# Kim-Dongjun/Soft-Truncation

Measured on AMD Instinct MI355X. Metric: training images/sec (DDPM++ CIFAR-10 32x32), higher is better.
Workload: dtype f32; 1 GPU; DDPM++ (VP) CIFAR-10 32x32, configs/vp/CIFAR10/ddpmpp_nll_st.py (BASELINE configs[1]); per_gpu_batch=128, global_batch=128, parallelism=dp1

## Files before the change

### soft-truncation_amd/csrc/conv.hip

```cpp
#include "igemm.h"
#include "stk_fp16.h"
#include "stk_fp16_train.h"

namespace {

using igemm::Cfg;
using igemm::MnMajor;
using igemm::keep_if;
using igemm::strip_row;

typedef __attribute__((address_space(1))) float gfloat;

struct ConvP {
  const float* x1; const float* x2; int C1, C2;
  const float* w; int w_layout;
  const float* bias; const float* temb; int temb_stride; const float* res; float inv_div; int use_div;
  float* y;
  const float* dy; float* dx1; float* dx2; float beta1, beta2, alpha;
  float* part; long part_stride;
  int N, H, W, Cin, Cout, OH, OW, KH, KW, stride, pad, sshift;
  int HW, OHW, taps;
  int ohw_shift, ow_shift;
};

// ... 561 lines not shown
  const bool al = stk_aligned16(p.part) && p.part_stride % 4 == 0 &&
                  (dgrad ? (p.HW % 4 == 0 && (!p.dx1 || stk_aligned16(p.dx1)) && (!p.dx2 || stk_aligned16(p.dx2)))
                         : (p.OHW % 4 == 0 && stk_aligned16(p.y) && (!p.res || stk_aligned16(p.res))));
  if (al && Ng % 4 == 0) {
    const dim3 rgrid((unsigned)stk_ew_grid((long)M * Ng / 4));
    if (dgrad) hipLaunchKernelGGL(slab_dgrad_kernel<4>, rgrid, dim3(256), 0, s, p, splits, M, (int)Ng);
    else hipLaunchKernelGGL(slab_fwd_kernel<4>, rgrid, dim3(256), 0, s, p, splits, M, (int)Ng);
  } else {
    const dim3 rgrid((unsigned)stk_ew_grid((long)M * Ng));
    if (dgrad) hipLaunchKernelGGL(slab_dgrad_kernel<1>, rgrid, dim3(256), 0, s, p, splits, M, (int)Ng);
    else hipLaunchKernelGGL(slab_fwd_kernel<1>, rgrid, dim3(256), 0, s, p, splits, M, (int)Ng);
  }
}

#include "conv_thin.h"
#include "conv_x2.h"
#include "conv_pl.h"
#include "conv_x2d.h"
#include "conv_x2w.h"

__device__ __forceinline__ long splitk_dst(long j, int layout, long CC, int Cout, int Cin, int taps) {
  if (layout == 0) {
    const int tap = (int)(j / CC);
    return (j - (long)tap * CC) * taps + tap;
  }
  const int co = (int)(j / Cin), ci = (int)(j - (long)co * Cin);
  return (long)ci * Cout + co;
}
__global__ __launch_bounds__(256) void splitk_reduce_kernel(const float* __restrict__ part, float* __restrict__ dw,
                                                            long n, int splits, long stride, float alpha, int layout,
                                                            int Cout, int Cin, int taps) {
  const long gstride = (long)gridDim.x * 256;
  const long CC = (long)Cout * Cin;
  const long n4 = ((n | stride) & 3) == 0 ? n / 4 : 0;
  for (long v = (long)blockIdx.x * 256 + threadIdx.x; v < n4; v += gstride) {
    const float4* src = reinterpret_cast<const float4*>(part) + v;
    float4 acc = {0.f, 0.f, 0.f, 0.f};
#pragma unroll 8
    for (int z = 0; z < splits; ++z) {
      const float4 t = src[(long)z * (stride / 4)];
      acc.x += t.x; acc.y += t.y; acc.z += t.z; acc.w += t.w;
    }
    const float a4[4] = {acc.x, acc.y, acc.z, acc.w};
#pragma unroll
    for (int e = 0; e < 4; ++e) dw[splitk_dst(4 * v + e, layout, CC, Cout, Cin, taps)] += alpha * a4[e];
  }
  for (long j = 4 * n4 + (long)blockIdx.x * 256 + threadIdx.x; j < n; j += gstride) {
    float sum = 0.f;
    for (int z = 0; z < splits; ++z) sum += part[(long)z * stride + j];
    dw[splitk_dst(j, layout, CC, Cout, Cin, taps)] += alpha * sum;
  }
}

__global__ __launch_bounds__(256) void splitk_reduce9_kernel(const float* __restrict__ part, float* __restrict__ dw, long CC,
                                                             int splits, long stride, float alpha) {
  __shared__ float s[256 * 9];
  const long q0 = (long)blockIdx.x * 256;
  const long q = q0 + threadIdx.x;
  const bool live = q < CC;
  float acc[9];
#pragma unroll
  for (int t = 0; t < 9; ++t) acc[t] = 0.f;
  const float* src = part + (live ? q : 0);
  int z = 0;
  for (; z + 4 <= splits; z += 4) {
    float v[4][9];
#pragma unroll
    for (int u = 0; u < 4; ++u)
#pragma unroll
      for (int t = 0; t < 9; ++t) v[u][t] = src[(long)(z + u) * stride + (long)t * CC];
#pragma unroll
    for (int u = 0; u < 4; ++u)
#pragma unroll
      for (int t = 0; t < 9; ++t) acc[t] += v[u][t];
  }
  for (; z < splits; ++z)
#pragma unroll
    for (int t = 0; t < 9; ++t) acc[t] += src[(long)z * stride + (long)t * CC];
#pragma unroll
  for (int t = 0; t < 9; ++t) s[threadIdx.x * 9 + t] = alpha * acc[t];
  __syncthreads();
  const long base = q0 * 9, end = CC * 9;
#pragma unroll
  for (int k = 0; k < 9; ++k) {
    const long i = base + k * 256 + threadIdx.x;
    if (i < end) dw[i] += s[k * 256 + threadIdx.x];
  }
}

template <int COLS>
__global__ __launch_bounds__(256) void wgrad9_kernel(ConvP p, int tiles_m, int tiles_n, int k_per_split) {
  constexpr int ROWS = 32 / COLS, TW = COLS + 2, TH = ROWS + 2, TSZ = TH * TW;
  constexpr int XS = TSZ | 1;
  constexpr int LDA = 129;
  constexpr int NX = (32 * TSZ + 255) / 256;
  constexpr int NA = 16;
  __shared__ float lds[32 * LDA + 32 * XS];
  float* As = lds;
  float* Xs = lds + 32 * LDA;

  const int tid = threadIdx.x, lane = tid & 63, wid = tid >> 6;
  const int fk = lane >> 5, fc = lane & 31;
  const int id = xcd_remap(blockIdx.x, gridDim.x);
  const int tn = id % tiles_n;
  const int rest = id / tiles_n;
  const int tm = rest % tiles_m, zs = rest / tiles_m;
// ... 252 lines not shown
    using A2 = std::conditional_t<X1, x2::ActLoader16<true, TAPS>, x2::ActLoader<true, TAPS>>;
    if (g.dual) hipLaunchKernelGGL((x2::gemm_kernel<A2, E>), g.grid, dim3(256), 0, g.s, g.p, g.q, g.M, g.Ng, g.tm, g.tn, g.nch,
                                   g.chunks_per_split, g.xpart, g.nx);
    else hipLaunchKernelGGL((x2::gemm_kernel<A1, E>), g.grid, dim3(256), 0, g.s, g.p, g.q, g.M, g.Ng, g.tm, g.tn, g.nch,
                            g.chunks_per_split, g.xpart, g.nx);
  } else if (g.halo) {
    if (g.p.W == 64)
      hipLaunchKernelGGL((x2d::gemm_halo_kernel<64, E, 1>), g.grid, dim3(256), 0, g.s, g.p, g.q, g.M, g.Ng, g.tm, g.tn, g.nch / 9, g.xpart, g.nx);
    else if (g.p.W == 32)
      hipLaunchKernelGGL((x2d::gemm_halo_kernel<32, E, 1>), g.grid, dim3(256), 0, g.s, g.p, g.q, g.M, g.Ng, g.tm, g.tn, g.nch / 9, g.xpart, g.nx);
    else
      hipLaunchKernelGGL((x2d::gemm_halo_kernel<16, E, 1>), g.grid, dim3(256), 0, g.s, g.p, g.q, g.M, g.Ng, g.tm, g.tn, g.nch / 9, g.xpart, g.nx);
  } else {
    hipLaunchKernelGGL((x2d::gemm_kernel<TAPS, 128, E>), g.grid, dim3(256), 0, g.s, g.p, g.q, g.M, g.Ng, g.tm, g.tn, g.nch,
                       g.chunks_per_split, g.xpart, g.nx);
  }
}
template <class E>
void split_gemm(const SplitGemm& g) {
  if (g.p.taps == 9) split_gemm_taps<E, 9>(g);
  else split_gemm_taps<E, 1>(g);
}

template <class EP>
int launch_split(ConvP p, const SplitPlan& r0, const float* s1, int S1, const float* s2, int S2, int M, long Ng, int dgrad,
                 void* ws, hipStream_t s, const void* wp_ready, float* amax, const void* planes, const float* planes_amax,
                 bool amax_valid, bool x1) {
  x2::Src q;
  q.s1 = s1; q.s2 = S2 > 0 ? s2 : s1; q.S1 = S1; q.S2 = S2; q.Kc = S1 + S2; q.Mpad = x2::pad128(M); q.taps = p.taps;
  q.pl = static_cast<const unsigned char*>(planes); q.pl_stride = planes ? pl::plane_bytes(p.N, S1, p.HW) : 0;
  const SplitWs lay = split_ws(r0, M, q.Kc, p.taps);
  unsigned char* base = reinterpret_cast<unsigned char*>(((uintptr_t)ws + 255) & ~(uintptr_t)255);
  float* xpart = reinterpret_cast<float*>(base + lay.xpart);
  p.part = reinterpret_cast<float*>(base + lay.part);
  p.part_stride = r0.slab;
  if (amax) xpart = amax + (dgrad ? 2 * x2::NPART : 0);
  if (planes) {
    xpart = const_cast<float*>(planes_amax);
  } else if (!(amax_valid && amax)) {
    hipLaunchKernelGGL(x2::amax_partial_kernel, dim3(x2::NPART), dim3(x2::AMAX_THREADS), 0, s, s1, (long)p.N * S1 * p.HW, xpart);
    if (S2 > 0)
      hipLaunchKernelGGL(x2::amax_partial_kernel, dim3(x2::NPART), dim3(x2::AMAX_THREADS), 0, s, s2, (long)p.N * S2 * p.HW,
                         xpart + x2::NPART);
    STK_CHECK_LAUNCH();
  }
  if (wp_ready) {
    q.wp = static_cast<const unsigned short*>(wp_ready);
  } else {
    x2::WprepDesc one = {};
    one.w = p.w; one.wp = base; one.M = M; one.Kc = q.Kc; one.Mpad = q.Mpad;
    one.taps = p.taps; one.flip = dgrad;
    split_weight_strides(p, dgrad, one.sm, one.sk);
    hipLaunchKernelGGL(x2::wamax_kernel, dim3(x2::WPART, 1), dim3(256), 0, s, nullptr, one);
    hipLaunchKernelGGL(x2::wprep_kernel, dim3((unsigned)stk_cdiv((long)q.Mpad * q.Kc, 256L)), dim3(256), 0, s, nullptr, one);
    STK_CHECK_LAUNCH();
    q.wp = reinterpret_cast<const unsigned short*>(base);
  }
  const int nch = planes && x1 ? p.taps * ((q.Kc / x2::KC + 1) / 2) : p.taps * (q.Kc / x2::KC);
  const SplitPlan r = planes && x1 ? x1_plan(r0, nch) : r0;
  SplitGemm g = {p, q, M, (int)Ng, q.Mpad / 128, stk_cdiv((int)Ng, 128), nch, r.chunks_per_split, xpart,
                 S2 > 0 ? 2 * x2::NPART : x2::NPART, S2 > 0, planes != nullptr, planes && x2d::halo_ok(p, p.taps, r0.splits),
                 dim3(), s};
  g.grid = dim3((unsigned)(g.tm * g.tn * r.splits));
  if (r0.splits == 1) {
    if (x1) split_gemm<OneProduct<EP>>(g);
    else split_gemm<EP>(g);
    STK_CHECK_LAUNCH();
    return STK_OK;
  }
  if (x1) split_gemm<OneProduct<EpSlab>>(g);
  else split_gemm<EpSlab>(g);
  STK_CHECK_LAUNCH();
  launch_slab_sum(p, r.splits, M, Ng, dgrad, s);
  STK_CHECK_LAUNCH();
  return STK_OK;
}

struct SplitWgradPlan { int ok; int splits; int chunks_per_split; long slab; int rows3; };
inline SplitWgradPlan split_wgrad_plan(int C1, int C2, int N, int Cout, int H, int W, int OH, int OW, int KH, int KW,
                                       int stride, int pad) {
  SplitWgradPlan q = {0, 0, 0, 0, 0};
  const int Cin = C1 + C2;
  const long K = (long)N * H * W;
  const int cmax = Cout > C1 ? (Cout > C2 ? Cout : C2) : (C1 > C2 ? C1 : C2);
  if (K * cmax * 4 >= 0x7fffffffL || (C2 > 0 && C1 % 32)) return q;
  const bool pow2 = (W & (W - 1)) == 0 && ((H * W) & (H * W - 1)) == 0;
  const bool geom = (KH == 3 && KW == 3 && pad == 1) || (KH == 1 && KW == 1 && pad == 0);
  if (!geom || stride != 1 || OH != H || OW != W || !pow2 || W < 4 || H * W < 16 || Cin < 64 || Cout < 64 ||
      K > 0x7fffffffL || K % 32)
    return q;
  const int taps = KH * KW;
  q.rows3 = (taps == 9 && W >= 8 && (C2 == 0 || C1 % 16 == 0)) ? 1 : 0;
  const long tiles = q.rows3 ? 3L * stk_cdiv(Cout, 128) * stk_cdiv(Cin, 64)
                             : (long)taps * stk_cdiv(Cout, 128) * stk_cdiv(Cin, 128);
  if (taps == 1 && tiles < 2) return q;
  const long chunks = K / 32;
  constexpr long w1_wgs = 256;
  long splits = (taps == 1 && tiles < 6 ? w1_wgs : 512) / tiles;
  if (splits > chunks / 8) splits = chunks / 8;
  if (splits < 1) splits = 1;
  q.chunks_per_split = (int)((chunks + splits - 1) / splits);
  q.splits = (int)((chunks + q.chunks_per_split - 1) / q.chunks_per_split);
  q.slab = (long)Cout * Cin * taps;
  q.ok = 1;
  return q;
}
template <int FORM>
// ... 480 lines not shown
                               false, f16x1);
}

int stk_conv2d_dgrad_pl_f32(const void* dypl, const float* dyamax, const float* w, int w_layout, float* dx1, int C1,
                            float beta1, float* dx2, int C2, float beta2, float alpha, int N, int H, int W, int Cout,
                            int KH, int KW, const void* wp, void* ws, long ws_bytes, void* stream) {
  return dgrad_pl_impl(dypl, dyamax, w, w_layout, dx1, C1, beta1, dx2, C2, beta2, alpha, N, H, W, Cout, KH, KW, wp, ws, ws_bytes,
                       stream, false);
}

int stk_conv2d_dgrad_pl_f16x1(const void* dypl, const float* dyamax, const float* w, int w_layout, float* dx1, int C1,
                              float beta1, float* dx2, int C2, float beta2, float alpha, int N, int H, int W, int Cout,
                              int KH, int KW, const void* wp, void* ws, long ws_bytes, void* stream) {
  return dgrad_pl_impl(dypl, dyamax, w, w_layout, dx1, C1, beta1, dx2, C2, beta2, alpha, N, H, W, Cout, KH, KW, wp, ws, ws_bytes,
                       stream, true);
}

int stk_conv2d_wgrad_pl_ok(int N, int H, int W, int Cin, int Cout) { return x2w::plan(N, H, W, Cin, Cout).ok; }

long stk_conv2d_wgrad_pl_ws_bytes(int N, int H, int W, int Cin, int Cout) {
  long m = 0;
  for (int wgs : {0, 256, 512, 768, 1024}) {
    const x2w::Plan q = x2w::plan(N, H, W, Cin, Cout, wgs);
    if (q.ok && (long)q.splits * q.slab > m) m = (long)q.splits * q.slab;
  }
  return m ? m * 4 + 256 : 0;
}

static int wgrad_pl_impl(const void* xpl, const float* xrec, const void* dypl, const float* dyrec, float* dw, float alpha,
                         float* ws, long ws_bytes, int N, int H, int W, int Cin, int Cout, int wgs, void* stream, bool f16x1) {
  if (!xpl || !xrec || !dypl || !dyrec || !dw || !ws || wgs < 0 || wgs > 1024) return STK_EINVAL;
  const x2w::Plan q = x2w::plan(N, H, W, Cin, Cout, wgs);
  if (!q.ok) return STK_EUNSUPPORTED;
  if (ws_bytes < (long)q.splits * q.slab * 4) return STK_EINVAL;
  x2w::Args a = {};
  a.dypl = static_cast<const unsigned char*>(dypl); a.dyrec = dyrec; a.dy_ps = pl::plane_bytes(N, Cout, H * W);
  a.xpl = static_cast<const unsigned char*>(xpl); a.xrec = xrec; a.x_ps = pl::plane_bytes(N, Cin, H * W);
  if (2 * a.dy_ps >= 0x7fffffffL || 2 * a.x_ps >= 0x7fffffffL) return STK_EUNSUPPORTED;
  a.part = ws; a.part_stride = q.slab;
  a.N = N; a.H = H; a.W = W; a.HW = H * W; a.Cin = Cin; a.Cout = Cout; a.Cob = Cout / 32; a.Cib = Cin / 32;
  a.tiles_co = stk_cdiv(Cout, 128); a.tiles_ci = Cin / 32;
  a.nchunks_total = (int)((long)N * H * W / 32); a.chunks_per_split = q.chunks_per_split;
  hipStream_t s = (hipStream_t)stream;
  const dim3 grid((unsigned)(a.tiles_co * a.tiles_ci * q.splits));
  if (f16x1) {
    if (q.groups == 2) launch_x2w<2 | x2w::X1_FORM>(a, W, grid, s);
    else launch_x2w<1 | x2w::X1_FORM>(a, W, grid, s);
  } else if (q.groups == 2) {
    launch_x2w<2>(a, W, grid, s);
  } else {
    launch_x2w<1>(a, W, grid, s);
  }
  STK_CHECK_LAUNCH();
  if (q.splits <= 64)
    hipLaunchKernelGGL(splitk_reduce9_kernel, dim3((unsigned)stk_cdiv((long)Cout * Cin, 256L)), dim3(256), 0, s, ws, dw, (long)Cout * Cin,
                       q.splits, q.slab, alpha);
  else
    hipLaunchKernelGGL(splitk_reduce_kernel, dim3(stk_ew_grid((q.slab + 3) / 4)), dim3(256), 0, s, ws, dw, q.slab, q.splits,
                       q.slab, alpha, 0, Cout, Cin, 9);
  STK_CHECK_LAUNCH();
  return STK_OK;
}

int stk_conv2d_wgrad_pl_f32(const void* xpl, const float* xrec, const void* dypl, const float* dyrec, float* dw,
                            float alpha, float* ws, long ws_bytes, int N, int H, int W, int Cin, int Cout, void* stream) {
  return stk_conv2d_wgrad_pl_wgs_f32(xpl, xrec, dypl, dyrec, dw, alpha, ws, ws_bytes, N, H, W, Cin, Cout, 0, stream);
}

int stk_conv2d_wgrad_pl_wgs_f32(const void* xpl, const float* xrec, const void* dypl, const float* dyrec, float* dw,
                                float alpha, float* ws, long ws_bytes, int N, int H, int W, int Cin, int Cout, int wgs, void* stream) {
  return wgrad_pl_impl(xpl, xrec, dypl, dyrec, dw, alpha, ws, ws_bytes, N, H, W, Cin, Cout, wgs, stream, false);
}

int stk_conv2d_wgrad_pl_f16x1(const void* xpl, const float* xrec, const void* dypl, const float* dyrec, float* dw,
                              float alpha, float* ws, long ws_bytes, int N, int H, int W, int Cin, int Cout, void* stream) {
  return wgrad_pl_impl(xpl, xrec, dypl, dyrec, dw, alpha, ws, ws_bytes, N, H, W, Cin, Cout, 0, stream, true);
}

int stk_conv2d_wgrad_pl_wgs_f16x1(const void* xpl, const float* xrec, const void* dypl, const float* dyrec, float* dw,
                                  float alpha, float* ws, long ws_bytes, int N, int H, int W, int Cin, int Cout, int wgs,
                                  void* stream) {
  return wgrad_pl_impl(xpl, xrec, dypl, dyrec, dw, alpha, ws, ws_bytes, N, H, W, Cin, Cout, wgs, stream, true);
}

int stk_conv2d_variant(int dir, int C1, int C2, int N, int H, int W, int Cout, int OH, int OW, int KH, int KW,
                       int stride, int pad, int w_layout) {
  ConvP p = {};
  if (fill_common(p, N, H, W, C1, C2, Cout, OH, OW, KH, KW, stride, pad)) return -1;
  const int Cin = C1 + C2;
  p.w_layout = w_layout;
  if (dir == 0) {
    const long Ng = (long)N * p.OHW;
    if (thin::geometry_ok(p) && ((C2 == 0 && Cin <= 4) || Cout <= 4)) return 4;
    if (fwd_split_plan(p).ok) return 5;
    return use_big_tile(Cout, Ng, 1) && !(p.taps == 1 && w_layout == 0 && (Cin % 8)) ? 1 : 0;
  }
  if (dir == 1) {
    const long Ng = (long)N * p.HW;
    if (thin::geometry_ok(p) && Cout <= 4) return 4;
    if (dgrad_split_plan(p).ok) return 5;
    return use_big_tile(Cin, Ng, 1) && !(p.taps == 1 && w_layout == 1 && (Cout % 8)) ? 1 : 0;
  }
  if (thin::geometry_ok(p) && ((C2 == 0 && Cin <= 4) || Cout <= 4)) return 4;
  if (split_wgrad_plan(C1, C2, N, Cout, H, W, OH, OW, KH, KW, stride, pad).ok) return 5;
  const bool can9 = stride == 1 && pad == 1 && C2 == 0 && OH == H && OW == W && w_layout == 0;
  const WgradPlan q = wgrad_plan(Cin, N, Cout, OH, OW, KH, KW, can9);
  return q.mode9 ? 3 : q.big;
}

long stk_conv2d_wp_bytes(int dir, int C1, int C2, int N, int H, int W, int Cout, int KH, int KW, int stride, int pad) {
  if (dir != 0 && dir != 1) return 0;
  if (stk_conv2d_variant(dir, C1, C2, N, H, W, Cout, H, W, KH, KW, stride, pad, 0) != 5) return 0;
  const int Cin = C1 + C2;
  return dir == 0 ? x2::wp_bytes(Cout, Cin, KH * KW) : x2::wp_bytes(Cin, Cout, KH * KW);
}

long stk_conv2d_wp_desc(int dir, const float* w, int w_layout, int Cin, int Cout, int KH, int KW, void* wp,
                        StkWprepDesc* out) {
  if (!w || !wp || !out || (dir != 0 && dir != 1) || (w_layout != 0 && w_layout != 1) || Cin <= 0 || Cout <= 0 ||
      (KH * KW != 9 && KH * KW != 1) || (w_layout == 1 && KH * KW != 1) || ((uintptr_t)wp & 255))
    return STK_EINVAL;
  ConvP p = {};
  p.Cin = Cin; p.Cout = Cout; p.taps = KH * KW; p.w_layout = w_layout;
  long sm, sk;
  split_weight_strides(p, dir, sm, sk);
  out->w = w; out->wp = wp; out->sm = sm; out->sk = sk;
  out->M = dir ? Cin : Cout; out->Kc = dir ? Cout : Cin; out->Mpad = x2::pad128(out->M); out->taps = p.taps;
  out->flip = dir; out->reserved = 0;
  return (long)out->Mpad * out->Kc;
}

int stk_conv2d_wprep_batch(const StkWprepDesc* descs_dev, int n, long max_items, void* stream) {
  static_assert(sizeof(StkWprepDesc) == sizeof(x2::WprepDesc), "descriptor layout");
  if (!descs_dev || n <= 0 || max_items <= 0 || n > 65535) return STK_EINVAL;
  const dim3 grid((unsigned)stk_cdiv(max_items, 256L), (unsigned)n);
  const x2::WprepDesc* d = reinterpret_cast<const x2::WprepDesc*>(descs_dev);
  hipLaunchKernelGGL(x2::wamax_kernel, dim3(x2::WPART, (unsigned)n), dim3(256), 0, (hipStream_t)stream, d, x2::WprepDesc{});
  hipLaunchKernelGGL(x2::wprep_kernel, grid, dim3(256), 0, (hipStream_t)stream, d, x2::WprepDesc{});
  STK_CHECK_LAUNCH();
  return STK_OK;
}

long stk_conv2d_fwd_ws_bytes(int C1, int C2, int N, int H, int W, int Cout, int KH, int KW, int stride, int pad) {
  ConvP p = {};
  if (fill_common(p, N, H, W, C1, C2, Cout, H, W, KH, KW, stride, pad)) return 0;
  return split_ws(fwd_split_plan(p), Cout, C1 + C2, p.taps).bytes;
}

long stk_conv2d_dgrad_ws_bytes(int C1, int C2, int N, int H, int W, int Cout, int KH, int KW, int stride, int pad) {
  ConvP p = {};
  if (fill_common(p, N, H, W, C1, C2, Cout, H, W, KH, KW, stride, pad)) return 0;
  return split_ws(dgrad_split_plan(p), C1 + C2, Cout, p.taps).bytes;
}

long stk_conv2d_wgrad_ws_bytes(int C1, int C2, int N, int Cout, int OH, int OW, int KH, int KW) {
  const WgradPlan a = wgrad_plan(C1 + C2, N, Cout, OH, OW, KH, KW, true);
  const WgradPlan b = wgrad_plan(C1 + C2, N, Cout, OH, OW, KH, KW, false);
  const SplitWgradPlan x = split_wgrad_plan(C1, C2, N, Cout, OH, OW, OH, OW, KH, KW, 1, KH == 3 ? 1 : 0);
  const long na = (long)a.splits * a.slab, nb = (long)b.splits * b.slab, nx = x.ok ? (long)x.splits * x.slab : 0;
  long m = na > nb ? na : nb;
  if (C2 == 0 && C1 <= 4) { const long t = (long)thin::wgrad_slabs(N, (long)OH * OW, Cout) * Cout * C1 * KH * KW; m = t > m ? t : m; }
  if (Cout <= 4) { const long t = (long)thin::wgrad_slabs(N, (long)OH * OW, C1 + C2) * Cout * (C1 + C2) * KH * KW; m = t > m ? t : m; }
  return (m > nx ? m : nx) * 4 + 256 + 256 + 3L * x2::NPART * 4;
}

int stk_gemm_f32(const float* A, long sam, long sak, long sab, const float* B, long sbk, long sbn, long sbb, float* C,
                 long scm, long scn, long scb, const float* bias, int bias_mode, int M, int N, int K, int batch,
                 float alpha, float beta, void* stream) {
  if (!A || !B || !C || M <= 0 || N <= 0 || K <= 0 || batch <= 0 || (bias_mode && !bias) || bias_mode < 0 ||
      bias_mode > 2)
    return STK_EINVAL;
  GemmP p;
  p.A = A; p.sam = sam; p.sak = sak; p.sab = sab; p.B = B; p.sbk = sbk; p.sbn = sbn; p.sbb = sbb;
  p.C = C; p.scm = scm; p.scn = scn; p.scb = scb; p.bias = bias; p.bias_mode = bias_mode;
  p.M = M; p.N = N; p.K = K; p.alpha = alpha; p.beta = beta;
  const bool ak = sak == 1 && (K % 8) == 0;
  const bool bk = sbk == 1 && sbn != 1 && (K % 8) == 0;
  const bool big = use_big_tile(M, N, batch);
  hipStream_t s = (hipStream_t)stream;
  using CB = Cfg<128, 128, 32>; using CS = Cfg<64, 64, 32>;
#define STK_GEMM_CASE(AK, BK)                                                                              \
  if (ak == AK && bk == BK) {                                                                              \
    if (big) return launch<CB, GemmP, GA<CB, AK>, GB<CB, BK>, EpGemm>(p, M, N, K, K, 1, batch, s);         \
    return launch<CS, GemmP, GA<CS, AK>, GB<CS, BK>, EpGemm>(p, M, N, K, K, 1, batch, s);                  \
  }
  STK_GEMM_CASE(true, true)
  STK_GEMM_CASE(true, false)
  STK_GEMM_CASE(false, true)
// ... 7 lines not shown
```

### soft-truncation_amd/csrc/conv_pl.h

```cpp
#pragma once

namespace pl {

using x2::HEADER;
using x2::NPART;
using x2::KC;
using x2::PITCH;
using x2::PLANE;

inline long plane_bytes(int N, int C, int HW) { return (long)N * ((C + 31) / 32) * HW * 64; }

constexpr int SP_PIX = 128;
__global__ __launch_bounds__(256) void split_planes_kernel(const float* __restrict__ x, int N, int C, int HW,
                                                           const float* __restrict__ amax, int namax,
                                                           unsigned char* __restrict__ out, long plane_stride) {
  __shared__ float t[32 * 129];
  __shared__ float red[4];
  const int tid = threadIdx.x;
  const int tiles = (HW + SP_PIX - 1) / SP_PIX;
  const int Cb = (C + 31) >> 5;
  const int tile = blockIdx.x % tiles, rest = blockIdx.x / tiles;
  const int cb = rest % Cb, n = rest / Cb;
  const int p0 = tile * SP_PIX;
  const bool vec = (HW & 3) == 0 && (reinterpret_cast<uintptr_t>(x) & 15) == 0;
#pragma unroll
  for (int k = 0; k < 4; ++k) {
    const int i = tid + 256 * k;
    const int c = i >> 5, q4 = i & 31;
    const int ch = cb * 32 + c, px = p0 + 4 * q4;
    float4 v = make_float4(0.f, 0.f, 0.f, 0.f);
    if (ch < C) {
      const float* src = x + ((long)n * C + ch) * HW + px;
      if (vec && px + 3 < HW) v = *reinterpret_cast<const float4*>(src);
      else {
        if (px < HW) v.x = src[0];
        if (px + 1 < HW) v.y = src[1];
        if (px + 2 < HW) v.z = src[2];
        if (px + 3 < HW) v.w = src[3];
      }
    }
    float* d = t + c * 129 + 4 * q4;
    d[0] = v.x; d[1] = v.y; d[2] = v.z; d[3] = v.w;
  }
  float m = 0.f;
  for (int i = tid; i < namax; i += 256) m = fmaxf(m, amax[i]);
  m = wave_max(m);
  if ((tid & 63) == 0) red[tid >> 6] = m;
  __syncthreads();
  const float s = x2::pow2_scale_of(fmaxf(fmaxf(red[0], red[1]), fmaxf(red[2], red[3])));
#pragma unroll
  for (int r = 0; r < 2; ++r) {
    const int id = tid + 256 * r;
    const int px = id >> 2, q = id & 3;
    unsigned hi[4], lo[4];
#pragma unroll
    for (int j = 0; j < 4; ++j) {
      const float v0 = s * t[(8 * q + 2 * j) * 129 + px], v1 = s * t[(8 * q + 2 * j + 1) * 129 + px];
      hi[j] = x2::pack_h2(v0, v1);
      lo[j] = x2::pack_h2(x2::lo_part(v0), x2::lo_part(v1));
    }
    if (p0 + px < HW) {
      unsigned char* o = out + (((long)n * Cb + cb) * HW + p0 + px) * 64 + q * 16;
      *reinterpret_cast<u32x4*>(o) = u32x4{hi[0], hi[1], hi[2], hi[3]};
      *reinterpret_cast<u32x4*>(o + plane_stride) = u32x4{lo[0], lo[1], lo[2], lo[3]};
    }
  }
}

}
```

### soft-truncation_amd/csrc/conv_x2.h

```cpp
#pragma once

typedef __attribute__((ext_vector_type(4))) unsigned u32x4;
typedef _Float16 halfx8 __attribute__((ext_vector_type(8)));
typedef _Float16 halfx2 __attribute__((ext_vector_type(2)));

namespace x2 {

constexpr int KC = 32;
constexpr int PITCH = 80;
constexpr int PLANE = 128 * PITCH;
constexpr int OPER = 2 * PLANE;
constexpr int LDS_BYTES = 2 * OPER;
constexpr int NPART = 256;
constexpr int HEADER = 256;

struct Src {
  const float* s1; const float* s2; int S1, S2;
  const unsigned short* wp; int Mpad; int Kc;
  int taps;
  const unsigned char* pl; long pl_stride;
};

__device__ __forceinline__ __amdgpu_buffer_rsrc_t make_rsrc(const void* base, long bytes) {
  return __builtin_amdgcn_make_buffer_rsrc(const_cast<void*>(base), 0, (int)bytes, 0x00020000);
// ... 59 lines not shown
  __device__ __forceinline__ float reduce(float* red, int tid) {
    const float v = wave_max(m);
    if ((tid & 63) == 0) red[tid >> 6] = v;
    __syncthreads();
    return fmaxf(fmaxf(red[0], red[1]), fmaxf(red[2], red[3]));
  }
};

__device__ __forceinline__ unsigned pack_h2(float lo, float hi) {
  const halfx2 v = {(_Float16)lo, (_Float16)hi};
  return __builtin_bit_cast(unsigned, v);
}
__device__ __forceinline__ float lo_part(float v) { return v - (float)(_Float16)v; }

struct WprepDesc {
  const float* w; unsigned char* wp; long sm, sk; int M, Kc, Mpad, taps, flip, reserved;
};
constexpr int WPART = 16;
__global__ __launch_bounds__(256) void wamax_kernel(const WprepDesc* __restrict__ descs, WprepDesc one) {
  __shared__ float red[4];
  const WprepDesc d = descs ? descs[blockIdx.y] : one;
  const long n = (long)d.M * d.Kc * d.taps;
  float m = 0.f;
  if ((reinterpret_cast<uintptr_t>(d.w) & 15) == 0) {
    const float4* w4 = reinterpret_cast<const float4*>(d.w);
    const long n4 = n >> 2;
    for (long i = (long)blockIdx.x * 1024 + threadIdx.x; i < n4; i += (long)WPART * 1024) {
      float4 v[4];
#pragma unroll
      for (int u = 0; u < 4; ++u) {
        const long j = i + 256 * u;
        v[u] = j < n4 ? w4[j] : make_float4(0.f, 0.f, 0.f, 0.f);
      }
#pragma unroll
      for (int u = 0; u < 4; ++u)
        m = fmaxf(m, fmaxf(fmaxf(fabsf(v[u].x), fabsf(v[u].y)), fmaxf(fabsf(v[u].z), fabsf(v[u].w))));
    }
    if (blockIdx.x == 0 && threadIdx.x < (n & 3)) m = fmaxf(m, fabsf(d.w[(n4 << 2) + threadIdx.x]));
  } else {
    for (long i = (long)blockIdx.x * 256 + threadIdx.x; i < n; i += (long)WPART * 256) m = fmaxf(m, fabsf(d.w[i]));
  }
  m = wave_max(m);
  if ((threadIdx.x & 63) == 0) red[threadIdx.x >> 6] = m;
  __syncthreads();
  if (threadIdx.x == 0) reinterpret_cast<float*>(d.wp)[blockIdx.x] = fmaxf(fmaxf(red[0], red[1]), fmaxf(red[2], red[3]));
}
__device__ __forceinline__ float weight_scale(const void* header) {
  const float* h = static_cast<const float*>(header);
  float m = 0.f;
#pragma unroll
  for (int i = 0; i < WPART; ++i) m = fmaxf(m, h[i]);
  return pow2_scale_of(m);
}
__global__ __launch_bounds__(256) void wprep_kernel(const WprepDesc* __restrict__ descs, WprepDesc one) {
  const WprepDesc d = descs ? descs[blockIdx.y] : one;
  const long total = (long)d.Mpad * d.Kc;
  const long i = (long)blockIdx.x * 256 + threadIdx.x;
  if (i >= total) return;
  const float s = weight_scale(d.wp);
  unsigned short* out = reinterpret_cast<unsigned short*>(d.wp + HEADER);
  const int kl = (int)(i & 31);
  const long rest = i >> 5;
  const int row = (int)(rest % d.Mpad), cc = (int)(rest / d.Mpad), k = cc * 32 + kl;
  const long plane = (long)d.taps * d.Mpad * d.Kc;
  const float* src = d.w + (row < d.M ? row * d.sm + k * d.sk : 0);
  for (int t = 0; t < d.taps; ++t) {
    const float a = row < d.M ? s * src[d.flip ? d.taps - 1 - t : t] : 0.f;
    const _Float16 h0 = (_Float16)a, h1 = (_Float16)(a - (float)h0);
    const long o = (((long)cc * d.taps + t) * d.Mpad + row) * 32 + kl;
    out[o] = __builtin_bit_cast(unsigned short, h0);
    out[plane + o] = __builtin_bit_cast(unsigned short, h1);
  }
}
inline long wp_bytes(int M, int Kc, int taps) { return HEADER + 2L * taps * pad128(M) * Kc * 2; }

template <bool X1>
struct Split16X {
  unsigned pk[2][8];
  __device__ __forceinline__ void st(int g, const float (&r)[16], float s, unsigned char* tile, int row, int k0,
                                     unsigned okm = 0xffffu) {
    if (g < 8) {
      const float v0 = s * igemm::keep_if(r[2 * g], okm, 2 * g), v1 = s * igemm::keep_if(r[2 * g + 1], okm, 2 * g + 1);
      pk[0][g] = pack_h2(v0, v1);
      if (!X1) pk[1][g] = pack_h2(lo_part(v0), lo_part(v1));
    } else if (g < 12) {
      const int sp = (g - 8) >> 1, h = (g - 8) & 1;
      if (X1 && sp) return;
      *reinterpret_cast<u32x4*>(tile + sp * PLANE + row * PITCH + k0 * 2 + h * 16) =
          u32x4{pk[sp][4 * h], pk[sp][4 * h + 1], pk[sp][4 * h + 2], pk[sp][4 * h + 3]};
    }
  }
};
using Split16 = Split16X<false>;

struct WpLoader {
  __amdgpu_buffer_rsrc_t rs; unsigned voff, plane2, chunk2; int row, seg;
  u32x4 r[4];
  __device__ __forceinline__ void init(const Src& q, int m0, int tid) {
    row = tid >> 2; seg = tid & 3;
    plane2 = (unsigned)q.taps * q.Mpad * q.Kc * 2u;
    chunk2 = (unsigned)q.Mpad * KC * 2u;
    rs = make_rsrc(reinterpret_cast<const unsigned char*>(q.wp) + HEADER, 2L * plane2);
    voff = ((unsigned)(m0 + row) * KC + seg * 8) * 2u;
  }
  __device__ __forceinline__ void ld(int g, int c) {
    if (g >= 4) return;
    r[g] = __builtin_bit_cast(u32x4, __builtin_amdgcn_raw_buffer_load_b128(
                                         rs, (int)voff, (int)((unsigned)c * chunk2 + (g >> 1) * plane2 + (g & 1) * 64u * KC * 2u), 0));
  }
  __device__ __forceinline__ void st(int g, unsigned char* t) {
    if (g < 4) *reinterpret_cast<u32x4*>(t + (g >> 1) * PLANE + (row + 64 * (g & 1)) * PITCH + seg * 16) = r[g];
  }
};

template <bool DUAL, int TAPS, bool X1>
struct ActLoaderT {
  __amdgpu_buffer_rsrc_t rs1, rs2;
  int nl, kg, tb1, tb2; unsigned mask; float scale;
  float r[16]; Split16X<X1> sp;
  __device__ __forceinline__ void init(const ConvP& p, const Src& q, int n0, int tid, float s) {
    nl = tid & 127;
    kg = __builtin_amdgcn_readfirstlane(tid >> 7);
    rs1 = make_rsrc(q.s1, (long)p.N * q.S1 * p.HW * 4);
    rs2 = make_rsrc(q.s2, (long)p.N * (DUAL ? q.S2 : q.S1) * p.HW * 4);
// ... 563 lines not shown
```

### soft-truncation_amd/csrc/reduce_optim.hip

```cpp
#include "common.h"

namespace {

__global__ __launch_bounds__(256) void softmax_fwd_kernel(const float* __restrict__ x, float* __restrict__ y,
                                                          long rows, int cols, float scale) {
  const int lane = threadIdx.x & 63;
  const long row = (long)blockIdx.x * 4 + (threadIdx.x >> 6);
  if (row >= rows) return;
  const float* p = x + row * cols;
  float* q = y + row * cols;
  float mx = -INFINITY;
  for (int i = lane; i < cols; i += 64) mx = fmaxf(mx, p[i] * scale);
  mx = wave_max(mx);
  float s = 0.f;
  for (int i = lane; i < cols; i += 64) {
    const float e = expf(p[i] * scale - mx);
    q[i] = e;
    s += e;
  }
  s = wave_sum(s);
  const float inv = 1.f / s;
  for (int i = lane; i < cols; i += 64) q[i] *= inv;
}

// ... 98 lines not shown
    const int n2 = n + 16;
    const long o0 = ((long)n * C + c) * HW, o1 = ((long)n2 * C + c) * HW;
    float s0 = row_sum_max<AMAX, RES>(dy + o0, HW, lane, vec, mx, RES ? res + o0 : nullptr, alpha, rbeta);
    float s1 = n2 < N ? row_sum_max<AMAX, RES>(dy + o1, HW, lane, vec, mx, RES ? res + o1 : nullptr, alpha, rbeta) : 0.f;
    s0 = alpha * wave_sum(s0);
    s1 = alpha * wave_sum(s1);
    if (rows && lane == 0) {
      rows[(long)n * rows_stride + c] = s0;
      if (n2 < N) rows[(long)n2 * rows_stride + c] = s1;
    }
    tot += s0;
    if (n2 < N) tot += s1;
  }
  if (AMAX) mx = wave_max(mx);
  if (lane == 0) { red[wv] = tot; if (AMAX) redm[wv] = mx; }
  __syncthreads();
  if (threadIdx.x == 0) {
    float t = 0.f;
#pragma unroll
    for (int q = 0; q < 16; ++q) t += red[q];
    if (dbias) dbias[c] += t;
    if (dbias2) dbias2[c] += t;
    if (AMAX) {
      float m = 0.f;
#pragma unroll
      for (int q = 0; q < 16; ++q) m = fmaxf(m, redm[q]);
      amax[c] = m;
      for (int i = c + C; i < 256; i += C) amax[i] = 0.f;
      if (amax2) {
        amax2[c] = m;
        for (int i = c + C; i < 256; i += C) amax2[i] = 0.f;
      }
    }
  }
}
__global__ __launch_bounds__(256) void colsum_acc_kernel(const float* __restrict__ src, float* __restrict__ dbias, int N,
                                                         int C, int stride) {
  __shared__ float red[256];
  const int cl = threadIdx.x & 31, part = threadIdx.x >> 5;
  const int c = blockIdx.x * 32 + cl;
  float s = 0.f;
  if (c < C)
    for (int n = part; n < N; n += 8) s += src[(long)n * stride + c];
  red[threadIdx.x] = s;
  __syncthreads();
  if (part == 0 && c < C) {
    float t = 0.f;
#pragma unroll
    for (int q = 0; q < 8; ++q) t += red[q * 32 + cl];
    dbias[c] += t;
  }
}

constexpr int SUMSQ_BLOCKS = 1024;
__global__ __launch_bounds__(256) void sumsq_stage1(const float* __restrict__ x, long n, float* __restrict__ part) {
  __shared__ float red[4];
  float s[1] = {0.f};
  const long stride = (long)gridDim.x * 256;
  if ((reinterpret_cast<uintptr_t>(x) & 15) == 0) {
    const long n4 = n >> 2;
    const float4* x4 = reinterpret_cast<const float4*>(x);
    for (long i = (long)blockIdx.x * 256 + threadIdx.x; i < n4; i += stride) {
      const float4 v = x4[i];
      s[0] += (v.x * v.x + v.y * v.y) + (v.z * v.z + v.w * v.w);
    }
    for (long i = (n4 << 2) + (long)blockIdx.x * 256 + threadIdx.x; i < n; i += stride) s[0] += x[i] * x[i];
  } else {
    for (long i = (long)blockIdx.x * 256 + threadIdx.x; i < n; i += stride) s[0] += x[i] * x[i];
  }
  block_sum<1>(s, red);
  if (threadIdx.x == 0) part[blockIdx.x] = s[0];
}
__global__ __launch_bounds__(256) void sumsq_stage2(const float* __restrict__ part, int nb, float* __restrict__ out) {
  __shared__ double red[4];
  double s = 0.0;
  for (int i = threadIdx.x; i < nb; i += 256) s += (double)part[i];
#pragma unroll
  for (int o = 32; o > 0; o >>= 1) s += __shfl_xor(s, o, 64);
  if ((threadIdx.x & 63) == 0) red[threadIdx.x >> 6] = s;
  __syncthreads();
  if (threadIdx.x == 0) out[0] = (float)(red[0] + red[1] + red[2] + red[3]);
}

struct AdamArgs {
  float lr, b1, b2, eps, wd, step_size, bc2_sqrt, max_norm;
  int adamw;
};
__device__ __forceinline__ void adam_one(float& p, float& g, float& m, float& v, const AdamArgs& a, float coef) {
  float gi = g * coef;
  g = gi;
  float pi = p;
  if (a.wd != 0.f) {
    if (a.adamw) pi = pi * (1.f - a.lr * a.wd);
    else gi = gi + a.wd * pi;
  }
  const float mi = m + (gi - m) * (1.f - a.b1);
  const float vi = v * a.b2 + (1.f - a.b2) * gi * gi;
  const float denom = sqrtf(vi) / a.bc2_sqrt + a.eps;
  p = pi - a.step_size * (mi / denom);
  m = mi;
  v = vi;
}
__global__ __launch_bounds__(256) void adam_kernel(float* __restrict__ p, float* __restrict__ g, float* __restrict__ m,
                                                   float* __restrict__ v, long n, AdamArgs a,
                                                   const float* __restrict__ sumsq) {
  float coef = 1.f;
// ... 89 lines not shown
  STK_CHECK_LAUNCH();
  return STK_OK;
}

int stk_softmax_bwd_f32(const float* y, const float* dy, float* dx, long rows, int cols, float scale, void* stream) {
  if (!y || !dy || !dx || rows <= 0 || cols <= 0) return STK_EINVAL;
  hipLaunchKernelGGL(softmax_bwd_kernel, dim3(stk_cdiv(rows, 4)), dim3(256), 0, S(stream), y, dy, dx, rows, cols, scale);
  STK_CHECK_LAUNCH();
  return STK_OK;
}

int stk_bias_grad_amax_f32(const float* dy, int N, int C, int HW, float alpha, float* dtemb, int temb_stride, float* dbias,
                           float* amax, float* ws, void* stream) {
  if (!dy || !amax || N <= 0 || C <= 0 || C > 256 || HW <= 0 || (!dtemb && !dbias && !ws)) return STK_EINVAL;
  if (HW < 4096) {
    hipLaunchKernelGGL(bias_grad_kernel<true>, dim3((unsigned)C), dim3(1024), 0, S(stream), dy, dtemb, temb_stride, dbias, N,
                       C, HW, alpha, amax);
    STK_CHECK_LAUNCH();
    return STK_OK;
  }
  if (dtemb || dbias) {
    const int rc = stk_bias_grad_f32(dy, N, C, HW, alpha, dtemb, temb_stride, dbias, ws, stream);
    if (rc) return rc;
  }
  return stk_amax_partial_f32(dy, (long)N * C * HW, amax, stream);
}

int stk_bias_grad_amax_res_f32(const float* dy, int N, int C, int HW, float alpha, float* dtemb, int temb_stride,
                               float* dbias, float* amax, float* dres, float dres_beta, float* ws, void* stream) {
  if (!dy || !amax || !dres || N <= 0 || C <= 0 || C > 256 || HW <= 0 || (!dtemb && !dbias && !ws)) return STK_EINVAL;
  if (HW < 4096) {
    hipLaunchKernelGGL((bias_grad_kernel<true, true>), dim3((unsigned)C), dim3(1024), 0, S(stream), dy, dtemb, temb_stride,
                       dbias, N, C, HW, alpha, amax, dres, dres_beta);
    STK_CHECK_LAUNCH();
    return STK_OK;
  }
  const int rc = stk_axpby_f32(dy, alpha, dres, dres_beta, dres, (long)N * C * HW, stream);
  if (rc) return rc;
  return stk_bias_grad_amax_f32(dy, N, C, HW, alpha, dtemb, temb_stride, dbias, amax, ws, stream);
}

int stk_bias_grad_amax_dual_f32(const float* dy, int N, int C, int HW, float alpha, float* dtemb, int temb_stride,
                                float* dbias, float* amax, float* dbias2, float* amax2, float* ws, void* stream) {
  if (!dy || !amax || !amax2 || N <= 0 || C <= 0 || C > 256 || HW <= 0 || HW >= 4096) return STK_EINVAL;
  hipLaunchKernelGGL((bias_grad_kernel<true, false>), dim3((unsigned)C), dim3(1024), 0, S(stream), dy, dtemb, temb_stride,
                     dbias, N, C, HW, alpha, amax, (float*)nullptr, 0.f, dbias2, amax2);
  STK_CHECK_LAUNCH();
  return STK_OK;
}

int stk_bias_grad_f32(const float* dy, int N, int C, int HW, float alpha, float* dtemb, int temb_stride, float* dbias,
                      float* ws, void* stream) {
  if (!dy || N <= 0 || C <= 0 || HW <= 0 || (!dtemb && !ws) || (!dtemb && !dbias)) return STK_EINVAL;
  if (dbias && HW < 4096) {
    hipLaunchKernelGGL(bias_grad_kernel<false>, dim3((unsigned)C), dim3(1024), 0, S(stream), dy, dtemb, temb_stride, dbias, N,
                       C, HW, alpha, (float*)nullptr);
    STK_CHECK_LAUNCH();
    return STK_OK;
  }
  float* rows = dtemb ? dtemb : ws;
  const int stride = dtemb ? temb_stride : C;
  if (HW >= 4096 && (HW & 3) == 0 && stk_aligned16(dy))
    hipLaunchKernelGGL(rowsum_block_kernel, dim3((unsigned)((long)N * C)), dim3(256), 0, S(stream), dy, rows, N, C, HW,
                       stride, alpha);
  else
    hipLaunchKernelGGL(rowsum_kernel, dim3(stk_cdiv((long)N * C, 4)), dim3(256), 0, S(stream), dy, rows, N, C, HW, stride,
                       alpha);
  STK_CHECK_LAUNCH();
  if (dbias) {
    hipLaunchKernelGGL(colsum_acc_kernel, dim3(stk_cdiv(C, 32)), dim3(256), 0, S(stream), rows, dbias, N, C, stride);
    STK_CHECK_LAUNCH();
  }
  return STK_OK;
}

int stk_sumsq_f32(const float* x, long n, float* out, float* ws, void* stream) {
  if (!x || !out || !ws || n < 0) return STK_EINVAL;
  int nb = stk_cdiv(n > 0 ? n : 1, 256L * 16);
  if (nb > SUMSQ_BLOCKS) nb = SUMSQ_BLOCKS;
  hipLaunchKernelGGL(sumsq_stage1, dim3(nb), dim3(256), 0, S(stream), x, n, ws);
  STK_CHECK_LAUNCH();
  hipLaunchKernelGGL(sumsq_stage2, dim3(1), dim3(256), 0, S(stream), ws, nb, out);
  STK_CHECK_LAUNCH();
  return STK_OK;
}

int stk_adam_f32(float* p, float* g, float* m, float* v, long n, float lr, float b1, float b2, float eps,
                 float weight_decay, int adamw, float bc1, float bc2, const float* sumsq, float max_norm,
                 void* stream) {
  if (!p || !g || !m || !v || n < 0 || bc1 == 0.f || bc2 <= 0.f) return STK_EINVAL;
  if (n == 0) return STK_OK;
  AdamArgs a;
  a.lr = lr; a.b1 = b1; a.b2 = b2; a.eps = eps; a.wd = weight_decay; a.adamw = adamw;
  a.step_size = lr / bc1;
  a.bc2_sqrt = sqrtf(bc2);
  a.max_norm = max_norm;
  const bool vec = stk_aligned16(p) && stk_aligned16(g) && stk_aligned16(m) && stk_aligned16(v);
  if (vec)
    hipLaunchKernelGGL(adam_kernel, dim3(stk_ew_grid(n >> 2 ? n >> 2 : 1)), dim3(256), 0, S(stream), p, g, m, v, n, a,
                       sumsq);
  else
    hipLaunchKernelGGL(adam_kernel_scalar, dim3(stk_ew_grid(n)), dim3(256), 0, S(stream), p, g, m, v, n, a, sumsq);
  STK_CHECK_LAUNCH();
  return STK_OK;
}

// ... 27 lines not shown
```

Baseline: 3450 images/s.

## Vectorize split-K reduce, tile weight prep through LDS, add HW=1 bias path

Adds a float4-vectorized split-K reduction for 3x3 weight gradients that uses smaller blocks and stages results in shared memory for coalesced dw updates. Rewrites the fp16 weight-prep kernel to process 1024 items per block, loading weights with vector reads into an LDS tile and writing packed hi/lo halves with 16-byte stores. It also batches loads ahead of stores in the plane-staging loop, and adds a dedicated column-sum kernel for bias gradients when HW is 1 (linear layers). These are small kernels, so end-to-end training throughput may change only slightly, and the more complex wprep path adds risk of layout bugs.

```diff
diff --git a/soft-truncation_amd/csrc/conv.hip b/soft-truncation_amd/csrc/conv.hip
--- a/soft-truncation_amd/csrc/conv.hip
+++ b/soft-truncation_amd/csrc/conv.hip
@@ -637,6 +637,41 @@
   }
 }
 
+constexpr int R9_PAIRS = 32;
+template <int U>
+__device__ __forceinline__ void reduce9_batch(const float4* __restrict__ src, long st4, int z, float4& acc) {
+  float4 v[U];
+#pragma unroll
+  for (int u = 0; u < U; ++u) v[u] = src[(long)(z + u) * st4];
+#pragma unroll
+  for (int u = 0; u < U; ++u) { acc.x += v[u].x; acc.y += v[u].y; acc.z += v[u].z; acc.w += v[u].w; }
+}
+__global__ __launch_bounds__(128) void splitk_reduce9v_kernel(const float* __restrict__ part, float* __restrict__ dw, long CC,
+                                                              int splits, long stride, float alpha) {
+  __shared__ float s[R9_PAIRS * 9];
+  const int tid = threadIdx.x;
+  const long q0 = (long)blockIdx.x * R9_PAIRS;
+  const int t = tid >> 3, c4 = (tid & 7) * 4;
+  if (t < 9 && q0 + c4 < CC) {
+    const float4* src = reinterpret_cast<const float4*>(part + (long)t * CC + q0 + c4);
+    const long st4 = stride >> 2;
+    float4 acc = {0.f, 0.f, 0.f, 0.f};
+    int z = 0;
+    for (; z + 16 <= splits; z += 16) reduce9_batch<16>(src, st4, z, acc);
+    for (; z + 4 <= splits; z += 4) reduce9_batch<4>(src, st4, z, acc);
+    for (; z < splits; ++z) reduce9_batch<1>(src, st4, z, acc);
+    s[(c4 + 0) * 9 + t] = alpha * acc.x;
+    s[(c4 + 1) * 9 + t] = alpha * acc.y;
+    s[(c4 + 2) * 9 + t] = alpha * acc.z;
+    s[(c4 + 3) * 9 + t] = alpha * acc.w;
+  }
+  __syncthreads();
+  const long base = q0 * 9, end = CC * 9;
+  for (int k = tid; k < R9_PAIRS * 9; k += 128) {
+    const long i = base + k;
+    if (i < end) dw[i] += s[k];
+  }
+}
 __global__ __launch_bounds__(256) void splitk_reduce9_kernel(const float* __restrict__ part, float* __restrict__ dw, long CC,
                                                              int splits, long stride, float alpha) {
   __shared__ float s[256 * 9];
@@ -995,7 +1030,7 @@
     one.taps = p.taps; one.flip = dgrad;
     split_weight_strides(p, dgrad, one.sm, one.sk);
     hipLaunchKernelGGL(x2::wamax_kernel, dim3(x2::WPART, 1), dim3(256), 0, s, nullptr, one);
-    hipLaunchKernelGGL(x2::wprep_kernel, dim3((unsigned)stk_cdiv((long)q.Mpad * q.Kc, 256L)), dim3(256), 0, s, nullptr, one);
+    hipLaunchKernelGGL(x2::wprep_kernel, dim3((unsigned)stk_cdiv((long)q.Mpad * q.Kc, (long)x2::WPREP_ITEMS)), dim3(256), 0, s, nullptr, one);
     STK_CHECK_LAUNCH();
     q.wp = reinterpret_cast<const unsigned short*>(base);
   }
@@ -1582,9 +1617,12 @@
     launch_x2w<1>(a, W, grid, s);
   }
   STK_CHECK_LAUNCH();
-  if (q.splits <= 64)
-    hipLaunchKernelGGL(splitk_reduce9_kernel, dim3((unsigned)stk_cdiv((long)Cout * Cin, 256L)), dim3(256), 0, s, ws, dw, (long)Cout * Cin,
-                       q.splits, q.slab, alpha);
+  const long CC = (long)Cout * Cin;
+  if (q.splits <= 64 && (CC & 3) == 0 && (q.slab & 3) == 0 && stk_aligned16(ws))
+    hipLaunchKernelGGL(splitk_reduce9v_kernel, dim3((unsigned)stk_cdiv(CC, (long)R9_PAIRS)), dim3(128), 0, s, ws, dw, CC, q.splits,
+                       q.slab, alpha);
+  else if (q.splits <= 64)
+    hipLaunchKernelGGL(splitk_reduce9_kernel, dim3((unsigned)stk_cdiv(CC, 256L)), dim3(256), 0, s, ws, dw, CC, q.splits, q.slab, alpha);
   else
     hipLaunchKernelGGL(splitk_reduce_kernel, dim3(stk_ew_grid((q.slab + 3) / 4)), dim3(256), 0, s, ws, dw, q.slab, q.splits,
                        q.slab, alpha, 0, Cout, Cin, 9);
@@ -1663,7 +1701,7 @@
 int stk_conv2d_wprep_batch(const StkWprepDesc* descs_dev, int n, long max_items, void* stream) {
   static_assert(sizeof(StkWprepDesc) == sizeof(x2::WprepDesc), "descriptor layout");
   if (!descs_dev || n <= 0 || max_items <= 0 || n > 65535) return STK_EINVAL;
-  const dim3 grid((unsigned)stk_cdiv(max_items, 256L), (unsigned)n);
+  const dim3 grid((unsigned)stk_cdiv(max_items, (long)x2::WPREP_ITEMS), (unsigned)n);
   const x2::WprepDesc* d = reinterpret_cast<const x2::WprepDesc*>(descs_dev);
   hipLaunchKernelGGL(x2::wamax_kernel, dim3(x2::WPART, (unsigned)n), dim3(256), 0, (hipStream_t)stream, d, x2::WprepDesc{});
   hipLaunchKernelGGL(x2::wprep_kernel, grid, dim3(256), 0, (hipStream_t)stream, d, x2::WprepDesc{});
diff --git a/soft-truncation_amd/csrc/conv_pl.h b/soft-truncation_amd/csrc/conv_pl.h
--- a/soft-truncation_amd/csrc/conv_pl.h
+++ b/soft-truncation_amd/csrc/conv_pl.h
@@ -23,24 +23,29 @@
   const int cb = rest % Cb, n = rest / Cb;
   const int p0 = tile * SP_PIX;
   const bool vec = (HW & 3) == 0 && (reinterpret_cast<uintptr_t>(x) & 15) == 0;
+  float4 v[4];
 #pragma unroll
   for (int k = 0; k < 4; ++k) {
     const int i = tid + 256 * k;
     const int c = i >> 5, q4 = i & 31;
     const int ch = cb * 32 + c, px = p0 + 4 * q4;
-    float4 v = make_float4(0.f, 0.f, 0.f, 0.f);
+    v[k] = make_float4(0.f, 0.f, 0.f, 0.f);
     if (ch < C) {
       const float* src = x + ((long)n * C + ch) * HW + px;
-      if (vec && px + 3 < HW) v = *reinterpret_cast<const float4*>(src);
+      if (vec && px + 3 < HW) v[k] = *reinterpret_cast<const float4*>(src);
       else {
-        if (px < HW) v.x = src[0];
-        if (px + 1 < HW) v.y = src[1];
-        if (px + 2 < HW) v.z = src[2];
-        if (px + 3 < HW) v.w = src[3];
+        if (px < HW) v[k].x = src[0];
+        if (px + 1 < HW) v[k].y = src[1];
+        if (px + 2 < HW) v[k].z = src[2];
+        if (px + 3 < HW) v[k].w = src[3];
       }
     }
-    float* d = t + c * 129 + 4 * q4;
-    d[0] = v.x; d[1] = v.y; d[2] = v.z; d[3] = v.w;
+  }
+#pragma unroll
+  for (int k = 0; k < 4; ++k) {
+    const int i = tid + 256 * k;
+    float* d = t + (i >> 5) * 129 + 4 * (i & 31);
+    d[0] = v[k].x; d[1] = v[k].y; d[2] = v[k].z; d[3] = v[k].w;
   }
   float m = 0.f;
   for (int i = tid; i < namax; i += 256) m = fmaxf(m, amax[i]);
diff --git a/soft-truncation_amd/csrc/conv_x2.h b/soft-truncation_amd/csrc/conv_x2.h
--- a/soft-truncation_amd/csrc/conv_x2.h
+++ b/soft-truncation_amd/csrc/conv_x2.h
@@ -135,12 +135,9 @@
   for (int i = 0; i < WPART; ++i) m = fmaxf(m, h[i]);
   return pow2_scale_of(m);
 }
-__global__ __launch_bounds__(256) void wprep_kernel(const WprepDesc* __restrict__ descs, WprepDesc one) {
-  const WprepDesc d = descs ? descs[blockIdx.y] : one;
-  const long total = (long)d.Mpad * d.Kc;
-  const long i = (long)blockIdx.x * 256 + threadIdx.x;
-  if (i >= total) return;
-  const float s = weight_scale(d.wp);
+constexpr int WPREP_ITEMS = 1024;
+constexpr int WPREP_TS = 32 * 32 + 4;
+__device__ __forceinline__ void wprep_item(const WprepDesc& d, float s, long i) {
   unsigned short* out = reinterpret_cast<unsigned short*>(d.wp + HEADER);
   const int kl = (int)(i & 31);
   const long rest = i >> 5;
@@ -153,6 +150,82 @@
     const long o = (((long)cc * d.taps + t) * d.Mpad + row) * 32 + kl;
     out[o] = __builtin_bit_cast(unsigned short, h0);
     out[plane + o] = __builtin_bit_cast(unsigned short, h1);
+  }
+}
+__global__ __launch_bounds__(256) void wprep_kernel(const WprepDesc* __restrict__ descs, WprepDesc one) {
+  __shared__ __attribute__((aligned(16))) unsigned tile[9 * WPREP_TS];
+  const WprepDesc d = descs ? descs[blockIdx.y] : one;
+  const long total = (long)d.Mpad * d.Kc;
+  const long i0 = (long)blockIdx.x * WPREP_ITEMS;
+  if (i0 >= total) return;
+  const int tid = threadIdx.x, taps = d.taps;
+  const float s = weight_scale(d.wp);
+  const bool by_k = d.sk == taps, by_row = d.sm == taps;
+  if ((d.Kc & 31) || (d.Mpad & 31) || taps > 9 || taps < 1 || !(by_k || by_row)) {
+    for (int u = 0; u < WPREP_ITEMS / 256; ++u) {
+      const long i = i0 + u * 256 + tid;
+      if (i < total) wprep_item(d, s, i);
+    }
+    return;
+  }
+  const long rest0 = i0 >> 5;
+  const int cc = (int)(rest0 / d.Mpad), r0 = (int)(rest0 - (long)cc * d.Mpad);
+  const int rv = d.M - r0 < 32 ? (d.M - r0 > 0 ? d.M - r0 : 0) : 32;
+  if (rv > 0) {
+    const float* __restrict__ base = d.w + (long)r0 * d.sm + (long)cc * 32 * d.sk;
+    const int nruns = by_k ? rv : 32, runlen = (by_k ? 32 : rv) * taps;
+    const long rstride = by_k ? d.sm : d.sk;
+    auto put = [&](int j, int e, float v) {
+      const int q = e / taps, ts = e - q * taps;
+      const int r = by_k ? j : q, kl = by_k ? q : j, t = d.flip ? taps - 1 - ts : ts;
+      const float a = s * v;
+      const _Float16 h0 = (_Float16)a, h1 = (_Float16)(a - (float)h0);
+      tile[t * WPREP_TS + r * 32 + kl] =
+          (unsigned)__builtin_bit_cast(unsigned short, h0) | ((unsigned)__builtin_bit_cast(unsigned short, h1) << 16);
+    };
+    if ((reinterpret_cast<uintptr_t>(base) & 15) == 0 && (rstride & 3) == 0 && (runlen & 3) == 0) {
+      const int rl4 = runlen >> 2, n4 = nruns * rl4;
+      for (int b = tid; b < n4; b += 256 * 3) {
+        float4 v[3];
+        int j[3], f[3];
+#pragma unroll
+        for (int u = 0; u < 3; ++u) {
+          const int idx = b + 256 * u;
+          j[u] = idx / rl4; f[u] = idx - j[u] * rl4;
+          if (idx < n4) v[u] = *reinterpret_cast<const float4*>(base + j[u] * rstride + 4 * f[u]);
+        }
+#pragma unroll
+        for (int u = 0; u < 3; ++u)
+          if (b + 256 * u < n4) {
+            put(j[u], 4 * f[u], v[u].x); put(j[u], 4 * f[u] + 1, v[u].y);
+            put(j[u], 4 * f[u] + 2, v[u].z); put(j[u], 4 * f[u] + 3, v[u].w);
+          }
+      }
+    } else {
+      const int n = nruns * runlen;
+      for (int idx = tid; idx < n; idx += 256) {
+        const int j = idx / runlen, e = idx - j * runlen;
+        put(j, e, base[j * rstride + e]);
+      }
+    }
+  }
+  __syncthreads();
+  unsigned short* out = reinterpret_cast<unsigned short*>(d.wp + HEADER);
+  const long plane = (long)taps * d.Mpad * d.Kc;
+  for (int p = tid; p < taps * 128; p += 256) {
+    const int kq = p & 3, r = (p >> 2) & 31, t = p >> 7;
+    const long o = (((long)cc * taps + t) * d.Mpad + r0 + r) * 32 + kq * 8;
+    u32x4 hi = {0u, 0u, 0u, 0u}, lo = {0u, 0u, 0u, 0u};
+    if (r < rv) {
+      const u32x4* src = reinterpret_cast<const u32x4*>(&tile[t * WPREP_TS + r * 32 + kq * 8]);
+      const u32x4 a = src[0], b = src[1];
+      hi = u32x4{(a[0] & 0xffffu) | (a[1] << 16), (a[2] & 0xffffu) | (a[3] << 16), (b[0] & 0xffffu) | (b[1] << 16),
+                 (b[2] & 0xffffu) | (b[3] << 16)};
+      lo = u32x4{(a[0] >> 16) | (a[1] & 0xffff0000u), (a[2] >> 16) | (a[3] & 0xffff0000u), (b[0] >> 16) | (b[1] & 0xffff0000u),
+                 (b[2] >> 16) | (b[3] & 0xffff0000u)};
+    }
+    *reinterpret_cast<u32x4*>(out + o) = hi;
+    *reinterpret_cast<u32x4*>(out + plane + o) = lo;
   }
 }
 inline long wp_bytes(int M, int Kc, int taps) { return HEADER + 2L * taps * pad128(M) * Kc * 2; }
diff --git a/soft-truncation_amd/csrc/reduce_optim.hip b/soft-truncation_amd/csrc/reduce_optim.hip
--- a/soft-truncation_amd/csrc/reduce_optim.hip
+++ b/soft-truncation_amd/csrc/reduce_optim.hip
@@ -174,6 +174,24 @@
   }
 }
 
+__global__ __launch_bounds__(256) void bias_cols_kernel(const float* __restrict__ dy, float* __restrict__ dbias, int N, int C,
+                                                        float alpha) {
+  __shared__ float red[256];
+  const int cl = threadIdx.x & 31, part = threadIdx.x >> 5;
+  const int c = blockIdx.x * 32 + cl;
+  float s = 0.f;
+  if (c < C)
+    for (int n = part; n < N; n += 8) s += alpha * dy[(long)n * C + c];
+  red[threadIdx.x] = s;
+  __syncthreads();
+  if (part == 0 && c < C) {
+    float t = 0.f;
+#pragma unroll
+    for (int q = 0; q < 8; ++q) t += red[q * 32 + cl];
+    dbias[c] += t;
+  }
+}
+
 constexpr int SUMSQ_BLOCKS = 1024;
 __global__ __launch_bounds__(256) void sumsq_stage1(const float* __restrict__ x, long n, float* __restrict__ part) {
   __shared__ float red[4];
@@ -369,6 +387,11 @@
 int stk_bias_grad_f32(const float* dy, int N, int C, int HW, float alpha, float* dtemb, int temb_stride, float* dbias,
                       float* ws, void* stream) {
   if (!dy || N <= 0 || C <= 0 || HW <= 0 || (!dtemb && !ws) || (!dtemb && !dbias)) return STK_EINVAL;
+  if (dbias && !dtemb && HW == 1) {
+    hipLaunchKernelGGL(bias_cols_kernel, dim3(stk_cdiv(C, 32)), dim3(256), 0, S(stream), dy, dbias, N, C, alpha);
+    STK_CHECK_LAUNCH();
+    return STK_OK;
+  }
   if (dbias && HW < 4096) {
     hipLaunchKernelGGL(bias_grad_kernel<false>, dim3((unsigned)C), dim3(1024), 0, S(stream), dy, dtemb, temb_stride, dbias, N,
                        C, HW, alpha, (float*)nullptr);
```

Result: no change. 3470 images/s, median of 6 (+0.6%).
